# RustCrypto/elliptic-curves

Hardware: NVIDIA H100
Metric: scalar-mults/sec (var-base, batch) at 1/2/4/8 H100 vs reference Rust CPU (higher is better)
Workload: dtype u32

## Files before the change

__graft_entry__.py:

```python
import os
import subprocess
import sys

ROOT = os.path.dirname(os.path.abspath(__file__))
PKG = os.path.join(ROOT, "elliptic-curves_b200")
CSRC = os.path.join(PKG, "csrc")
LIB = os.path.join(PKG, "libecgpu.so")
NVCC_FLAGS = [
    "-gencode", "arch=compute_90a,code=sm_90a", "-O3", "-lineinfo", "-std=c++17",
    "-Xcompiler", "-fPIC",
]
CURVE_GROUPS = (0, 1, 2, 3, 4, 5, 6)


def _newer(target, sources):
    if not os.path.exists(target):
        return True
    t = os.path.getmtime(target)
    return any(os.path.getmtime(s) > t for s in sources)


def _paths():
    for p in (ROOT, PKG, os.path.join(ROOT, "oracle"), os.path.join(ROOT, "tests")):
        if p not in sys.path:
            sys.path.insert(0, p)


def _build_dev(nvcc, srcs, force):
    dev_dir = os.path.join(ROOT, "tests", "dev")
    src = os.path.join(dev_dir, "fe_dev.cu")
    dev_so, sim_so = os.path.join(dev_dir, "libecgdev.so"), os.path.join(dev_dir, "libecgdevsim.so")
    if force or _newer(sim_so, srcs + [src]):
        subprocess.check_call(["g++", "-O2", "-std=c++17", "-Wno-unknown-pragmas", "-shared", "-fPIC", "-x", "c++", "-o", sim_so, src])
    if force or _newer(dev_so, srcs + [src]):
        objdir = os.path.join(dev_dir, "_build")
        os.makedirs(objdir, exist_ok=True)
        procs, objs = [], []
        for part in ("0", "1", "2", "3", "4", None):
            obj = os.path.join(objdir, f"fe_dev_s{part}.o" if part else "fe_dev_main.o")
            cmd = [nvcc] + NVCC_FLAGS + ["-Xcompiler", "-fvisibility=hidden"] + ([f"-DDEV_SHAPE={part}"] if part else []) + ["-c", "-o", obj, src]
            print("[build]", " ".join(cmd), flush=True)
            procs.append((cmd, subprocess.Popen(cmd)))
            objs.append(obj)
        for cmd, pr in procs:
            if pr.wait() != 0:
                raise subprocess.CalledProcessError(pr.returncode, cmd)
        subprocess.check_call([nvcc, "-shared", "-o", dev_so] + objs)
    x_src = os.path.join(dev_dir, "x448_dev.cu")
    x_so, x_sim = os.path.join(dev_dir, "libecgx448dev.so"), os.path.join(dev_dir, "libecgx448devsim.so")
    if force or _newer(x_sim, srcs + [x_src]):
        subprocess.check_call(["g++", "-O2", "-std=c++17", "-Wno-unknown-pragmas", "-shared", "-fPIC", "-x", "c++", "-o", x_sim, x_src])
    if force or _newer(x_so, srcs + [x_src]):
        cmd = [nvcc] + NVCC_FLAGS + ["-Xcompiler", "-fvisibility=hidden", "-shared", "-o", x_so, x_src]
        print("[build]", " ".join(cmd), flush=True)
        subprocess.check_call(cmd)
    e_src = os.path.join(dev_dir, "ed448_dev.cu")
    e_so, e_sim = os.path.join(dev_dir, "libecged448dev.so"), os.path.join(dev_dir, "libecged448devsim.so")
    if force or _newer(e_sim, srcs + [e_src]):
        subprocess.check_call(["g++", "-O2", "-std=c++17", "-Wno-unknown-pragmas", "-shared", "-fPIC", "-x", "c++", "-o", e_sim, e_src])
    if force or _newer(e_so, srcs + [e_src]):
        cmd = [nvcc] + NVCC_FLAGS + ["-Xcompiler", "-fvisibility=hidden", "-shared", "-o", e_so, e_src]
        print("[build]", " ".join(cmd), flush=True)
        subprocess.check_call(cmd)
    g_src = os.path.join(dev_dir, "ed448_group_dev.cu")
    g_so, g_sim = os.path.join(dev_dir, "libecged448gdev.so"), os.path.join(dev_dir, "libecged448gdevsim.so")
    if force or _newer(g_sim, srcs + [g_src]):
        subprocess.check_call(["g++", "-O2", "-std=c++17", "-Wno-unknown-pragmas", "-shared", "-fPIC", "-x", "c++", "-o", g_sim, g_src])
    if force or _newer(g_so, srcs + [g_src]):
        cmd = [nvcc] + NVCC_FLAGS + ["-Xcompiler", "-fvisibility=hidden", "-shared", "-o", g_so, g_src]
        print("[build]", " ".join(cmd), flush=True)
        subprocess.check_call(cmd)


def build(force: bool = False) -> None:
    nvcc = os.environ.get("NVCC", "/usr/local/cuda/bin/nvcc")
    srcs = [os.path.join(CSRC, f) for f in sorted(os.listdir(CSRC))] + [os.path.join(ROOT, "include", "ecgpu.h")]
    if force or _newer(LIB, srcs):
        objdir = os.path.join(PKG, "_build")
        os.makedirs(objdir, exist_ok=True)
        procs, objs = [], []
        for g in CURVE_GROUPS:
            obj = os.path.join(objdir, f"ecgpu_tu{g}.o")
            cmd = [nvcc] + NVCC_FLAGS + [f"-DECG_TU={g}", "-c", "-o", obj, os.path.join(CSRC, "ecgpu.cu")]
            print("[build]", " ".join(cmd), flush=True)
            procs.append((cmd, subprocess.Popen(cmd)))
            objs.append(obj)
        for cmd, pr in procs:
            if pr.wait() != 0:
                raise subprocess.CalledProcessError(pr.returncode, cmd)
        cmd = [nvcc, "-shared", "-o", LIB] + objs
        print("[build]", " ".join(cmd), flush=True)
        subprocess.check_call(cmd)
    _paths()
    import ecref

    ecref.build(force)
    sim_dir = os.path.join(ROOT, "tests", "sim")
    sim_so = os.path.join(sim_dir, "libecgsim.so")
    if force or _newer(sim_so, srcs + [os.path.join(sim_dir, "sim.cpp")]):
        subprocess.check_call(["g++", "-O2", "-std=c++17", "-Wno-unknown-pragmas", "-shared", "-fPIC", "-pthread", "-o", sim_so,
                               os.path.join(sim_dir, "sim.cpp")])
    _build_dev(nvcc, srcs, force)
    import ecgpu

    ecgpu.load_library()


def smoke() -> None:
    _paths()
    if not os.path.exists(LIB):
        build()
    import numpy as np

    import ecgpu
    import ecref
    import pyref
    from helpers import pack_points, pack_scalars, random_points

    eng = ecgpu.Engine([0])
    for curve in ("k256", "p256"):
        c = pyref.CURVES[curve]
        n = 257
# ... 38 lines not shown
```

elliptic-curves_b200/csrc/ecg_fe_k256.cuh:

```cuda
#pragma once
#include "ecg_prim.cuh"

namespace ecg {

#ifndef ECG_K256_OPT
#define ECG_K256_OPT 7
#endif
#if defined(__CUDA_ARCH__) || defined(__CUDACC__)
#define ECG_NOINLINE_D __device__ __noinline__
#else
#define ECG_NOINLINE_D
#endif

template <int OPT>
struct FpK256T {
  static constexpr int NL = 8;
  static constexpr bool LE = false;
  static constexpr int FB = 32;
  typedef FeN<8> FeT;
  typedef JacN<8> JacT;
  typedef AffN<8> AffT;
  static constexpr uint32_t C0 = 977u;
  static constexpr bool SQR_TRADE_DBL = (OPT & 64) != 0;
  static constexpr bool SQR_TRADE_MADD = (OPT & 128) != 0;
  static constexpr bool DBL_CALL = (OPT & 2048) != 0;
  static constexpr bool MADD_CALL = (OPT & 4096) != 0;
  static constexpr bool DBL_3M5S = false;
  typedef FpK256T<(OPT & (1 | 8 | 64 | 128))> Inline;

  ECG_D static void set_zero(Fe& r) {
#pragma unroll
    for (int i = 0; i < 8; i++) r.v[i] = 0;
  }
  ECG_D static void set_one(Fe& r) {
    set_zero(r);
    r.v[0] = 1;
  }

  ECG_D static void fold_top(uint32_t* r, uint32_t t0, uint32_t t1) {
    uint32_t q0, q1;
    mul_wide(q0, q1, t0, C0);
    uint64_t s1 = (uint64_t)q1 + t0 + (t1 ? C0 : 0u);
    uint32_t p1 = (uint32_t)s1;
    uint32_t p2 = (uint32_t)(s1 >> 32) + t1;
    r[0] = add_cc(r[0], q0);
    r[1] = addc_cc(r[1], p1);
    r[2] = addc_cc(r[2], p2);
#pragma unroll
    for (int i = 3; i < 8; i++) r[i] = addc_cc(r[i], 0);
    uint32_t cf = addc(0, 0);
    r[0] = add_cc(r[0], cf ? C0 : 0u);
    r[1] = addc_cc(r[1], cf);
    r[2] = addc_cc(r[2], 0);
    r[3] = addc(r[3], 0);
  }

  ECG_D static void reduce16(Fe& r, const uint32_t* t) {
    uint32_t lo[8], q[8];
#pragma unroll
    for (int i = 0; i < 8; i++) {
      lo[i] = t[i];
      q[i] = t[8 + i];
    }
    mad_wide_cc(lo[0], lo[1], t[8], C0);
    madc_wide_cc(lo[2], lo[3], t[10], C0);
    madc_wide_cc(lo[4], lo[5], t[12], C0);
    madc_wide_cc(lo[6], lo[7], t[14], C0);
    uint32_t e8 = addc(0, 0);
    mad_wide_cc(q[0], q[1], t[9], C0);
    madc_wide_cc(q[2], q[3], t[11], C0);
    madc_wide_cc(q[4], q[5], t[13], C0);
    madc_wide_cc(q[6], q[7], t[15], C0);
    uint32_t q8 = addc(0, 0);
    r.v[0] = lo[0];
    r.v[1] = add_cc(lo[1], q[0]);
#pragma unroll
    for (int k = 2; k < 8; k++) r.v[k] = addc_cc(lo[k], q[k - 1]);
    uint32_t t0 = addc_cc(e8, q[7]);
    uint32_t t1 = addc(q8, 0);
    fold_top(r.v, t0, t1);
  }

  ECG_D static void mul_body(Fe& r, const Fe& a, const Fe& b) {
    uint32_t t[16];
    if (OPT & 8)
      mul8x8_kara(t, a.v, b.v);
    else
      mul8x8(t, a.v, b.v);
    reduce16(r, t);
  }
  ECG_D static void sqr_body(Fe& r, const Fe& a) {
    uint32_t t[16];
    if (OPT & 1)
      sqr8(t, a.v);
    else
      mul8x8(t, a.v, a.v);
    reduce16(r, t);
  }
  static ECG_NOINLINE_D Fe mul_call(Fe a, Fe b) {
    Fe r;
    mul_body(r, a, b);
    return r;
  }
  static ECG_NOINLINE_D void mul_call_mem(Fe* r, const Fe* a, const Fe* b) {
    Fe x = *a, y = *b, z;
    mul_body(z, x, y);
    *r = z;
  }
  static ECG_NOINLINE_D void sqr_call_mem(Fe* r, const Fe* a) {
    Fe x = *a, z;
    sqr_body(z, x);
    *r = z;
  }
  static ECG_NOINLINE_D Fe sqr_call(Fe a) {
    Fe r;
    sqr_body(r, a);
    return r;
  }
  ECG_D static void mul(Fe& r, const Fe& a, const Fe& b) {
    if (OPT & 256)
      mul_call_mem(&r, &a, &b);
    else if (OPT & 2)
      r = mul_call(a, b);
    else
      mul_body(r, a, b);
  }
  ECG_D static void mul_d(Fe& r, const Fe& a, const Fe& b) {
    if (OPT & 256)
      mul_call_mem(&r, &a, &b);
    else if ((OPT & 2) && !(OPT & 32))
      r = mul_call(a, b);
    else
      mul_body(r, a, b);
// ... 67 lines not shown
  ECG_D static bool is_zero(const Fe& a) {
    uint32_t o = a.v[0] | a.v[1] | a.v[2] | a.v[3] | a.v[4] | a.v[5] | a.v[6] | a.v[7];
    uint32_t n = (a.v[0] ^ 0xFFFFFC2Fu) | (a.v[1] ^ 0xFFFFFFFEu) | ~(a.v[2] & a.v[3] & a.v[4] & a.v[5] & a.v[6] & a.v[7]);
    return (o == 0) | (n == 0);
  }
  ECG_D static bool is_canonical(const Fe& a) {
    uint32_t hi = a.v[2] & a.v[3] & a.v[4] & a.v[5] & a.v[6] & a.v[7];
    bool ge = (hi == 0xFFFFFFFFu) && (a.v[1] == 0xFFFFFFFFu || (a.v[1] == 0xFFFFFFFEu && a.v[0] >= 0xFFFFFC2Fu));
    return !ge;
  }
  ECG_D static void sqr_n(Fe& r, const Fe& a, int n) {
    r = a;
#pragma unroll 1
    for (int i = 0; i < n; i++) sqr(r, r);
  }
  ECG_D static void inv(Fe& r, const Fe& a) {
    Fe x2, x3, x6, x9, x11, x22, x44, x88, x176, x220, x223, t;
    sqr(x2, a);
    mul(x2, x2, a);
    sqr(x3, x2);
    mul(x3, x3, a);
    sqr_n(x6, x3, 3);
    mul(x6, x6, x3);
    sqr_n(x9, x6, 3);
    mul(x9, x9, x3);
    sqr_n(x11, x9, 2);
    mul(x11, x11, x2);
    sqr_n(x22, x11, 11);
    mul(x22, x22, x11);
    sqr_n(x44, x22, 22);
    mul(x44, x44, x22);
    sqr_n(x88, x44, 44);
    mul(x88, x88, x44);
    sqr_n(x176, x88, 88);
    mul(x176, x176, x88);
    sqr_n(x220, x176, 44);
    mul(x220, x220, x44);
    sqr_n(x223, x220, 3);
    mul(x223, x223, x3);
    sqr_n(t, x223, 23);
    mul(t, t, x22);
    sqr_n(t, t, 5);
    mul(t, t, a);
    sqr_n(t, t, 3);
    mul(t, t, x2);
    sqr_n(t, t, 2);
    mul(r, t, a);
  }
  ECG_D static void from_canonical(Fe& r, const Fe& a) { r = a; }
  ECG_D static void to_canonical(Fe& r, const Fe& a) { normalize(r, a); }
};

typedef FpK256T<ECG_K256_OPT> FpK256;

}
```

elliptic-curves_b200/csrc/ecg_fe_mont.cuh:

```cuda
#pragma once
#include "ecg_prim.cuh"

namespace ecg {

#ifndef ECG_NOINLINE_D
#if defined(__CUDA_ARCH__) || defined(__CUDACC__)
#define ECG_NOINLINE_D __device__ __noinline__
#else
#define ECG_NOINLINE_D
#endif
#endif

template <class PR, bool CALLS = true>
struct FpMontT {
  static constexpr int NL = PR::NL;
  typedef PR Params;
  typedef FeN<NL> FeT;
  typedef JacN<NL> JacT;
  typedef AffN<NL> AffT;
  typedef FeT Fe;
  static constexpr bool MONT = true;
  static constexpr bool LE = PR::LE;
  static constexpr int FB = PR::FB;
  static constexpr bool SQR_TRADE_DBL = false;
  static constexpr bool SQR_TRADE_MADD = false;
  static constexpr bool DBL_CALL = false;
  static constexpr bool MADD_CALL = false;
  static constexpr bool DBL_3M5S = false;
  typedef FpMontT<PR, CALLS> Inline;

  ECG_D static void set_zero(Fe& r) {
#pragma unroll
    for (int i = 0; i < NL; i++) r.v[i] = 0;
  }
  ECG_D static void set_one(Fe& r) {
#pragma unroll
    for (int i = 0; i < NL; i++) r.v[i] = PR::ONE(i);
  }

  ECG_D static void cond_sub_p(Fe& r, const uint32_t* t, uint32_t carry) {
    uint32_t u[NL];
    u[0] = sub_cc(t[0], PR::P(0));
#pragma unroll
    for (int i = 1; i < NL; i++) u[i] = subc_cc(t[i], PR::P(i));
    uint32_t bw = 0u - subc(0u, 0u);
    bool take = (carry != 0) | (bw == 0);
#pragma unroll
    for (int i = 0; i < NL; i++) r.v[i] = take ? u[i] : t[i];
  }

  ECG_D static void redc_mersenne(Fe& r, const uint32_t* u) {
    constexpr int B = PR::MERSENNE, W = B / 32, S = B % 32, K = 32 * NL - B;
    static_assert(PR::MERSENNE == 0 || (W == NL - 1 && S > 0 && K == 32 - S), "one partial top limb");
    constexpr uint32_t TOPMASK = (1u << S) - 1u;
    uint32_t lo[NL], hi[NL], v[NL];
#pragma unroll
    for (int i = 0; i < W; i++) lo[i] = u[i];
    lo[W] = u[W] & TOPMASK;
#pragma unroll
    for (int i = 0; i < NL; i++) hi[i] = (u[W + i] >> S) | ((W + i + 1 < 2 * NL ? u[W + i + 1] : 0u) << K);
    addN<NL>(v, lo, hi);
    const uint32_t c = v[W] >> S;
    v[W] &= TOPMASK;
    v[0] = add_cc(v[0], c);
#pragma unroll
    for (int i = 1; i < NL - 1; i++) v[i] = addc_cc(v[i], 0u);
    v[NL - 1] = addc(v[NL - 1], 0u);
    Fe w;
    cond_sub_p(w, v, 0u);
    const uint32_t low = w.v[0] & ((1u << K) - 1u);
#pragma unroll
    for (int i = 0; i < W; i++) r.v[i] = (w.v[i] >> K) | (w.v[i + 1] << S);
    r.v[W] = 0;
    constexpr int POS = B - K, PL = POS / 32, PS = POS % 32;
    r.v[PL] |= low << PS;
    if (PS + K > 32) r.v[PL + 1] |= low >> (32 - PS);
  }
  ECG_D static void mul_full(uint32_t* u, const Fe& a, const Fe& b) {
// ... 211 lines not shown
```

elliptic-curves_b200/csrc/ecg_fe_p256.cuh:

```cuda
#pragma once
#include "ecg_prim.cuh"

namespace ecg {

#ifndef ECG_P256_OPT
#define ECG_P256_OPT 515
#endif
#ifndef ECG_NOINLINE_D
#if defined(__CUDA_ARCH__) || defined(__CUDACC__)
#define ECG_NOINLINE_D __device__ __noinline__
#else
#define ECG_NOINLINE_D
#endif
#endif

template <int OPT>
struct FpP256T {
  static constexpr int NL = 8;
  static constexpr bool LE = false;
  static constexpr int FB = 32;
  typedef FeN<8> FeT;
  typedef JacN<8> JacT;
  typedef AffN<8> AffT;
  static constexpr bool SQR_TRADE_DBL = false;
  static constexpr bool SQR_TRADE_MADD = false;
  static constexpr bool DBL_CALL = (OPT & 2048) != 0;
  static constexpr bool MADD_CALL = (OPT & 4096) != 0;
  static constexpr bool DBL_3M5S = (OPT & 1024) != 0;
  typedef FpP256T<(OPT & (1 | 8 | 16 | 512 | 1024))> Inline;
  ECG_D static void set_zero(Fe& r) {
#pragma unroll
    for (int i = 0; i < 8; i++) r.v[i] = 0;
  }
  static constexpr bool MONT = (OPT & 512) != 0;
  ECG_D static void set_one(Fe& r) {
    set_zero(r);
    r.v[0] = 1;
    if (MONT) {
      r.v[3] = r.v[4] = r.v[5] = 0xFFFFFFFFu;
      r.v[6] = 0xFFFFFFFEu;
    }
  }

  ECG_D static uint32_t add_K(uint32_t* r, uint32_t c) {
    uint32_t m = 0u - c;
    r[0] = add_cc(r[0], c);
    r[1] = addc_cc(r[1], 0);
    r[2] = addc_cc(r[2], 0);
    r[3] = addc_cc(r[3], m);
    r[4] = addc_cc(r[4], m);
    r[5] = addc_cc(r[5], m);
    r[6] = addc_cc(r[6], m & 0xFFFFFFFEu);
    r[7] = addc_cc(r[7], 0);
    return addc(0, 0);
  }
  ECG_D static uint32_t sub_K(uint32_t* r, uint32_t c) {
    uint32_t m = 0u - c;
    r[0] = sub_cc(r[0], c);
    r[1] = subc_cc(r[1], 0);
    r[2] = subc_cc(r[2], 0);
    r[3] = subc_cc(r[3], m);
    r[4] = subc_cc(r[4], m);
    r[5] = subc_cc(r[5], m);
    r[6] = subc_cc(r[6], m & 0xFFFFFFFEu);
    r[7] = subc_cc(r[7], 0);
    return 0u - subc(0, 0);
  }

  ECG_D static int32_t fold_signed(uint32_t* r, int32_t o) {
    int64_t t = (int64_t)r[0] + o;
    r[0] = (uint32_t)t;
    t >>= 32;
    t += r[1];
    r[1] = (uint32_t)t;
    t >>= 32;
    t += r[2];
    r[2] = (uint32_t)t;
    t >>= 32;
// ... 360 lines not shown
```

elliptic-curves_b200/csrc/ecg_fe_p384.cuh:

```cuda
#pragma once
#include "ecg_prim.cuh"

namespace ecg {

#ifndef ECG_P384_OPT
#define ECG_P384_OPT 2
#endif
#ifndef ECG_NOINLINE_D
#if defined(__CUDA_ARCH__) || defined(__CUDACC__)
#define ECG_NOINLINE_D __device__ __noinline__
#else
#define ECG_NOINLINE_D
#endif
#endif

template <int OPT>
struct FpP384T {
  static constexpr int NL = 12;
  static constexpr bool LE = false;
  static constexpr int FB = 48;
  typedef FeN<12> FeT;
  typedef JacN<12> JacT;
  typedef AffN<12> AffT;
  typedef FeT Fe;
  static constexpr bool MONT = false;
  static constexpr bool SQR_TRADE_DBL = false;
  static constexpr bool SQR_TRADE_MADD = false;
  static constexpr bool DBL_CALL = false;
  static constexpr bool MADD_CALL = false;
  static constexpr bool DBL_3M5S = false;
  typedef FpP384T<0> Inline;

  ECG_D static void set_zero(Fe& r) {
#pragma unroll
    for (int i = 0; i < 12; i++) r.v[i] = 0;
  }
  ECG_D static void set_one(Fe& r) {
    set_zero(r);
    r.v[0] = 1;
  }

  ECG_D static uint32_t add_oK(uint32_t* r, uint32_t o) {
    uint32_t m = o ? 0xFFFFFFFFu : 0u;
    r[0] = add_cc(r[0], o);
    r[1] = addc_cc(r[1], 0u - o);
    r[2] = addc_cc(r[2], m);
    r[3] = addc_cc(r[3], (o - 1u) & m);
    r[4] = addc_cc(r[4], o);
#pragma unroll
    for (int i = 5; i < 12; i++) r[i] = addc_cc(r[i], 0u);
    return addc(0u, 0u);
  }
  ECG_D static uint32_t sub_K(uint32_t* r, uint32_t c) {
    uint32_t m = 0u - c;
    r[0] = sub_cc(r[0], c);
    r[1] = subc_cc(r[1], m);
    r[2] = subc_cc(r[2], m);
    r[3] = subc_cc(r[3], 0u);
    r[4] = subc_cc(r[4], c);
#pragma unroll
    for (int i = 5; i < 12; i++) r[i] = subc_cc(r[i], 0u);
    return 0u - subc(0u, 0u);
  }

  ECG_D static void acc_add(uint32_t* acc, const uint32_t* v) {
    acc[0] = add_cc(acc[0], v[0]);
#pragma unroll
    for (int i = 1; i < 12; i++) acc[i] = addc_cc(acc[i], v[i]);
    acc[12] = addc(acc[12], 0u);
  }
  ECG_D static void acc_sub(uint32_t* acc, const uint32_t* v) {
    acc[0] = sub_cc(acc[0], v[0]);
#pragma unroll
    for (int i = 1; i < 12; i++) acc[i] = subc_cc(acc[i], v[i]);
    acc[12] = subc(acc[12], 0u);
  }

  ECG_D static void reduce24(Fe& r, const uint32_t* c) {
    uint32_t acc[13], v[12];
    acc[0] = add_cc(c[0], 0xFFFFFFFCu);
// ... 186 lines not shown
```

elliptic-curves_b200/csrc/ecg_kernels.cuh:

```cuda
#pragma once
#if defined(__CUDACC__)
#include <cuda_runtime.h>
#else
#ifndef ECG_HOST_SIM
#error "ecg_kernels.cuh is CUDA code; a host build exists only for the test simulation (tests/sim/sim.cpp)"
#endif
#endif

#include "../../include/ecgpu.h"
#include "ecg_curves.cuh"
#include "ecg_io.cuh"
#include "ecg_mul.cuh"
#include "ecg_verify.cuh"

using namespace ecg;

#define ERRF_SCALAR 1u
#define ERRF_POINT 2u
#define ERRF_SKEW 4u

ECG_DEV void report_error(uint32_t* status, uint32_t flag, size_t idx) {
  atomicOr(&status[0], flag);
  atomicMin(&status[1], (uint32_t)(idx > 0xFFFFFFFEull ? 0xFFFFFFFEull : idx));
}

template <int NW>
ECG_DEV void soa_store(uint32_t* buf, size_t n, size_t idx, const uint32_t* v, int w0) {
#pragma unroll
  for (int w = 0; w < NW; w++) buf[(size_t)(w0 + w) * n + idx] = v[w];
}
template <int NW>
ECG_DEV void soa_load(uint32_t* v, const uint32_t* buf, size_t n, size_t idx, int w0) {
#pragma unroll
  for (int w = 0; w < NW; w++) v[w] = buf[(size_t)(w0 + w) * n + idx];
}

template <class C>
ECG_DEV uint32_t load_pair(uint32_t* k, typename C::F::AffT& P, bool& inf, const uint8_t* kb,
                                              const uint8_t* pxy, const uint8_t* pinf, size_t idx) {
  typedef typename C::F F;
  typedef typename F::FeT Fe;
  constexpr int NL = F::NL, FB = F::FB;
  uint32_t err = 0;
  load_fe<F>(k, kb + FB * idx);
  if (!ltN<NL>(k, C::N())) err |= ERRF_SCALAR;
  inf = pinf != nullptr && pinf[idx] != 0;
  Fe x, y;
  load_fe<F>(x.v, pxy + 2 * FB * idx);
  load_fe<F>(y.v, pxy + 2 * FB * idx + FB);
  if (!inf) {
    bool ok = ltN<NL>(x.v, C::P()) && ltN<NL>(y.v, C::P());
    F::from_canonical(P.x, x);
    F::from_canonical(P.y, y);
    if (ok) {
      Fe b;
      C::b_internal(b);
      ok = aff_on_curve<F, C::A_IS_MINUS3>(P, b);
    }
    if (!ok) err |= ERRF_POINT;
  }
  if (inf || err) {
    C::generator(P);
#pragma unroll
    for (int i = 0; i < NL; i++) k[i] = (i == 0);
  }
  return err;
}

#define K_TAB_WORDS 128
#define P_TAB_WORDS 192

typedef FpK256T<1> FpK256Inline;
template <int BLOCK, int MINBLK>
ECG_KERNEL(BLOCK, MINBLK)
    k256_varbase_kernel(const uint8_t* __restrict__ kb, const uint8_t* __restrict__ pxy,
                        const uint8_t* __restrict__ pinf, size_t n, uint32_t* __restrict__ jac,
                        uint32_t* __restrict__ gtab, uint32_t* __restrict__ status, size_t base) {
  size_t idx = (size_t)blockIdx.x * BLOCK + threadIdx.x;
  const bool live = idx < n;
  const size_t cidx = live ? idx : n - 1;
  uint32_t k[8];
  Aff P;
  bool inf;
  uint32_t err = load_pair<CurveK256>(k, P, inf, kb, pxy, pinf, cidx);
  if (err && live) report_error(status, err, base + idx);
  TabRef tab{gtab + (size_t)blockIdx.x * BLOCK * K_TAB_WORDS + threadIdx.x, (uint32_t)BLOCK};
  Jac r;
  k256_mul_thread<FpK256Inline, 1>(r, k, P, tab);
  if (!live) return;
  if (inf || err) FpK256::set_zero(r.Z);
  soa_store<8>(jac, n, idx, r.X.v, 0);
  soa_store<8>(jac, n, idx, r.Y.v, 8);
  soa_store<8>(jac, n, idx, r.Z.v, 16);
}

template <class C>
ECG_DEV uint32_t load_pair_or_generator(uint32_t* k, typename C::F::AffT& P, bool& inf, const uint8_t* kb, const uint8_t* pxy,
                                        const uint8_t* pinf, size_t idx) {
  typedef typename C::F F;
  if (pxy != nullptr) return load_pair<C>(k, P, inf, kb, pxy, pinf, idx);
  inf = false;
  load_fe<F>(k, kb + F::FB * idx);
  C::generator(P);
  if (ltN<F::NL>(k, C::N())) return 0;
#pragma unroll
  for (int i = 0; i < F::NL; i++) k[i] = (i == 0);
  return ERRF_SCALAR;
}

template <int BLOCK, int MINBLK>
ECG_KERNEL(BLOCK, MINBLK)
    k256_varbase_ct_kernel(const uint8_t* __restrict__ kb, const uint8_t* __restrict__ pxy, const uint8_t* __restrict__ pinf, size_t n,
                           uint32_t* __restrict__ jac, uint32_t* __restrict__ gtab, uint32_t* __restrict__ status, size_t base) {
  size_t idx = (size_t)blockIdx.x * BLOCK + threadIdx.x;
  if (idx >= n) return;
  uint32_t k[8];
  Aff P;
  bool inf;
  uint32_t err = load_pair_or_generator<CurveK256>(k, P, inf, kb, pxy, pinf, idx);
  if (err) report_error(status, err, base + idx);
  TabRef tab{gtab + (size_t)blockIdx.x * BLOCK * K_TAB_WORDS + threadIdx.x, (uint32_t)BLOCK};
  Jac r;
  k256_mul_thread<FpK256, 0, true>(r, k, P, tab);
  if (inf || err) FpK256::set_zero(r.Z);
  soa_store<8>(jac, n, idx, r.X.v, 0);
  soa_store<8>(jac, n, idx, r.Y.v, 8);
  soa_store<8>(jac, n, idx, r.Z.v, 16);
}

template <class C, int BLOCK, int MINBLK, bool CT = false>
ECG_KERNEL(BLOCK, MINBLK)
    generic_varbase_kernel(const uint8_t* __restrict__ kb, const uint8_t* __restrict__ pxy,
                           const uint8_t* __restrict__ pinf, size_t n, uint32_t* __restrict__ jac,
                           uint32_t* __restrict__ gtab, uint32_t* __restrict__ status, size_t base) {
  typedef typename C::F F;
  constexpr int NL = F::NL;
  size_t idx = (size_t)blockIdx.x * BLOCK + threadIdx.x;
  if (idx >= n) return;
  uint32_t k[NL];
// ... 1007 lines not shown
```

elliptic-curves_b200/csrc/ecg_mul.cuh:

```cuda
#pragma once
#include "ecg_fe_k256.cuh"
#include "ecg_point.cuh"
#include "ecg_scalar.cuh"

namespace ecg {

template <int NL>
struct TabRefN {
  uint32_t* base;
  uint32_t stride;
  ECG_D void store(int e, const FeN<NL>& x, const FeN<NL>& y) const {
#pragma unroll
    for (int w = 0; w < NL; w++) {
      base[(e * 2 * NL + w) * stride] = x.v[w];
      base[(e * 2 * NL + NL + w) * stride] = y.v[w];
    }
  }
  ECG_D void load(int e, FeN<NL>& x, FeN<NL>& y) const {
#pragma unroll
    for (int w = 0; w < NL; w++) {
      x.v[w] = base[(e * 2 * NL + w) * stride];
      y.v[w] = base[(e * 2 * NL + NL + w) * stride];
    }
  }
  ECG_D void load_ct(uint32_t idx, FeN<NL>& x, FeN<NL>& y) const {
#pragma unroll
    for (int w = 0; w < NL; w++) x.v[w] = y.v[w] = 0;
#pragma unroll 1
    for (uint32_t e = 0; e < 8; e++) {
      const uint32_t m = 0u - (uint32_t)(e == idx);
#pragma unroll
      for (int w = 0; w < NL; w++) {
        x.v[w] |= base[(e * 2 * NL + w) * stride] & m;
        y.v[w] |= base[(e * 2 * NL + NL + w) * stride] & m;
      }
    }
  }
};
typedef TabRefN<8> TabRef;
template <int NL>
struct TabRefJN {
  uint32_t* base;
  uint32_t stride;
  ECG_D void store(int e, const JacN<NL>& p) const {
#pragma unroll
    for (int w = 0; w < NL; w++) {
      base[(e * 3 * NL + w) * stride] = p.X.v[w];
      base[(e * 3 * NL + NL + w) * stride] = p.Y.v[w];
      base[(e * 3 * NL + 2 * NL + w) * stride] = p.Z.v[w];
    }
  }
  ECG_D void load(int e, JacN<NL>& p) const {
#pragma unroll
    for (int w = 0; w < NL; w++) {
      p.X.v[w] = base[(e * 3 * NL + w) * stride];
      p.Y.v[w] = base[(e * 3 * NL + NL + w) * stride];
      p.Z.v[w] = base[(e * 3 * NL + 2 * NL + w) * stride];
    }
  }
  ECG_D void load_ct(uint32_t idx, JacN<NL>& p) const {
#pragma unroll
    for (int w = 0; w < NL; w++) p.X.v[w] = p.Y.v[w] = p.Z.v[w] = 0;
#pragma unroll 1
    for (uint32_t e = 0; e < 8; e++) {
      const uint32_t m = 0u - (uint32_t)(e == idx);
#pragma unroll
      for (int w = 0; w < NL; w++) {
        p.X.v[w] |= base[(e * 3 * NL + w) * stride] & m;
        p.Y.v[w] |= base[(e * 3 * NL + NL + w) * stride] & m;
        p.Z.v[w] |= base[(e * 3 * NL + 2 * NL + w) * stride] & m;
      }
    }
  }
};
typedef TabRefJN<8> TabRefJ;

ECG_D void k256_beta(Fe& b) {
  const uint32_t B[8] = {0x719501EEu, 0xC1396C28u, 0x12F58995u, 0x9CF04975u, 0xAC3434E9u, 0x6E64479Eu, 0x657C0710u, 0x7AE96A2Bu};
#pragma unroll
  for (int i = 0; i < 8; i++) b.v[i] = B[i];
}

template <class F>
ECG_D void build_table_iso_a0(const TabRef& tab, Fe& Zg, const Aff& P) {
  Jac d, cur;
  aff_dbl<F, false>(d, P);
  Fe z2, z3;
  F::sqr(z2, d.Z);
  F::mul(z3, z2, d.Z);
  F::mul(cur.X, P.x, z2);
  F::mul(cur.Y, P.y, z3);
  F::set_one(cur.Z);
  Aff dd;
  dd.x = d.X;
  dd.y = d.Y;
  Fe zr[8];
  tab.store(0, cur.X, cur.Y);
#pragma unroll 1
  for (int i = 1; i < 8; i++) {
    jac_madd<F, false>(cur, cur, dd, &zr[i]);
    tab.store(i, cur.X, cur.Y);
  }
  F::mul(Zg, cur.Z, d.Z);
  Fe zs = zr[7];
#pragma unroll 1
  for (int i = 6; i >= 0; i--) {
    Fe x, y, zz;
    tab.load(i, x, y);
    F::sqr(zz, zs);
    F::mul(x, x, zz);
    F::mul(zz, zz, zs);
    F::mul(y, y, zz);
    tab.store(i, x, y);
    if (i > 0) F::mul(zs, zs, zr[i]);
  }
}

#if defined(__CUDA_ARCH__)
#define ECG_BLOCK_SYNC() __syncthreads()
#else
#define ECG_BLOCK_SYNC() ((void)0)
#endif
template <class F = FpK256, int PHASE_SYNC = 0, bool CT = false>
ECG_D void k256_mul_thread(Jac& r, const uint32_t* k, const Aff& P, const TabRef& tab) {
  GlvHalf g1, g2;
  glv_split_k256<CT>(g1, g2, k);
  Fe Zg, beta;
  build_table_iso_a0<F>(tab, Zg, P);
  k256_beta(beta);

  Jac acc;
  Aff e;
  tab.load(0, acc.X, acc.Y);
  fe_cneg<F>(acc.Y, g1.neg);
  F::set_one(acc.Z);
  tab.load(0, e.x, e.y);
  F::mul(e.x, e.x, beta);
  fe_cneg<F>(e.y, g2.neg);
  jac_madd<F, false>(acc, acc, e);

#pragma unroll 1
  for (int i = 0; i < 32; i++) {
    if (PHASE_SYNC == 1) ECG_BLOCK_SYNC();
#pragma unroll 1
    for (int j = 0; j < 4; j++) {
      if (PHASE_SYNC == 2) ECG_BLOCK_SYNC();
      jac_dbl<F, false>(acc, acc);
    }
    if (PHASE_SYNC == 1) ECG_BLOCK_SYNC();
#pragma unroll 1
    for (int half = 0; half < 2; half++) {
      if (PHASE_SYNC == 2) ECG_BLOCK_SYNC();
      uint32_t n = half ? next_window(g2.h) : next_window(g1.h);
      uint32_t sneg = half ? g2.neg : g1.neg;
      uint32_t pos = n >> 3;
      uint32_t idx = pos ? (n & 7u) : (7u - n);
      if (CT)
        tab.load_ct(idx, e.x, e.y);
      else
        tab.load((int)idx, e.x, e.y);
      if (half) F::mul(e.x, e.x, beta);
      fe_cneg<F>(e.y, (pos ^ sneg) ^ 1u);
      jac_madd<F, false>(acc, acc, e);
    }
  }
#pragma unroll 1
  for (int half = 0; half < 2; half++) {
    uint32_t ev = half ? g2.even : g1.even;
    uint32_t sneg = half ? g2.neg : g1.neg;
    tab.load(0, e.x, e.y);
    if (half) F::mul(e.x, e.x, beta);
    fe_cneg<F>(e.y, sneg ^ 1u);
    Jac t;
    jac_madd<F, false>(t, acc, e);
    jac_csel(acc, t, ev);
  }
  r.X = acc.X;
  r.Y = acc.Y;
  F::mul(r.Z, acc.Z, Zg);
}

template <class F, int A_IS_MINUS3, int PHASE_SYNC = 0, bool CT = false>
ECG_D void generic_mul_thread(typename F::JacT& r, const uint32_t* k, const typename F::AffT& P, const TabRefJN<F::NL>& tab) {
  typedef typename F::JacT Jac;
  typedef typename F::AffT Aff;
  FullRecodeN<F::NL> rc;
  recode_full<F::NL>(rc, k);
  Jac d, cur, acc;
  aff_dbl<F, A_IS_MINUS3>(d, P);
  cur.X = P.x;
  cur.Y = P.y;
  F::set_one(cur.Z);
  acc = cur;
  tab.store(0, cur);
  jac_madd<F, A_IS_MINUS3>(cur, d, P);
  tab.store(1, cur);
#pragma unroll 1
  for (int i = 2; i < 8; i++) {
    jac_add<F, A_IS_MINUS3>(cur, cur, d);
    tab.store(i, cur);
  }
#pragma unroll 1
  for (int i = 0; i < F::NL * 8; i++) {
#pragma unroll 1
    for (int j = 0; j < 4; j++) {
      if (PHASE_SYNC == 2) ECG_BLOCK_SYNC();
      jac_dbl<F, A_IS_MINUS3>(acc, acc);
    }
    if (PHASE_SYNC == 2) ECG_BLOCK_SYNC();
    uint32_t n = next_windowN<F::NL>(rc.h);
    uint32_t pos = n >> 3;
    uint32_t idx = pos ? (n & 7u) : (7u - n);
    Jac e;
    if (CT)
      tab.load_ct(idx, e);
    else
      tab.load((int)idx, e);
    fe_cneg<F>(e.Y, pos ^ 1u);
    jac_add<F, A_IS_MINUS3>(acc, acc, e);
  }
  Aff np;
  np.x = P.x;
  F::neg(np.y, P.y);
  Jac t;
// ... 7 lines not shown
```

elliptic-curves_b200/csrc/ecg_point.cuh:

```cuda
#pragma once
#include "ecg_prim.cuh"

namespace ecg {

typedef JacN<8> Jac;
typedef AffN<8> Aff;

template <class F>
ECG_D void fe_cneg(typename F::FeT& a, uint32_t c) {
  typename F::FeT n;
  F::neg(n, a);
#pragma unroll
  for (int i = 0; i < F::NL; i++) a.v[i] = c ? n.v[i] : a.v[i];
}
template <int NL>
ECG_D void jac_csel(JacN<NL>& r, const JacN<NL>& t, uint32_t c) {
#pragma unroll
  for (int i = 0; i < NL; i++) {
    r.X.v[i] = c ? t.X.v[i] : r.X.v[i];
    r.Y.v[i] = c ? t.Y.v[i] : r.Y.v[i];
    r.Z.v[i] = c ? t.Z.v[i] : r.Z.v[i];
  }
}

template <class F, int A_IS_MINUS3>
ECG_D void jac_dbl_body(typename F::JacT& r, const typename F::JacT& p) {
  typedef typename F::FeT Fe;
  Fe A, L, T, D, t, zz;
  F::sqr(A, p.Y);
  if (A_IS_MINUS3 == 1) {
    Fe u, v;
    F::sqr(zz, p.Z);
    F::sub(u, p.X, zz);
    F::add(v, p.X, zz);
    F::mul_d(L, u, v);
  } else {
    F::sqr(L, p.X);
  }
  F::sqr(D, A);
  if (A_IS_MINUS3 == 0 && F::SQR_TRADE_DBL) {
    F::add(t, p.X, A);
    F::sqr(T, t);
    F::sub(T, T, L);
    F::sub(T, T, D);
    F::half(T, T);
  } else {
    F::mul_d(T, p.X, A);
  }
  F::mul_small(L, L, 3);
  if constexpr (A_IS_MINUS3 == 2) {
    Fe z4, ca;
    F::sqr(zz, p.Z);
    F::sqr(z4, zz);
    F::curve_a(ca);
    F::mul_d(z4, z4, ca);
    F::add(L, L, z4);
  }
  F::half(L, L);
  if (A_IS_MINUS3 == 1 && F::DBL_3M5S) {
    Fe s2;
    F::add(s2, p.Y, p.Z);
    F::sqr(s2, s2);
    F::sub(s2, s2, A);
    F::sub(s2, s2, zz);
    F::half(r.Z, s2);
  } else {
    F::mul_d(r.Z, p.Y, p.Z);
  }
  F::sqr(r.X, L);
  F::add(t, T, T);
  F::sub(r.X, r.X, t);
  F::sub(t, T, r.X);
  F::mul_d(r.Y, L, t);
  F::sub(r.Y, r.Y, D);
}

#if defined(__CUDA_ARCH__) || defined(__CUDACC__)
#define ECG_NOINLINE_PT __device__ __noinline__
#else
#define ECG_NOINLINE_PT
#endif
template <class F, int A_IS_MINUS3>
ECG_NOINLINE_PT typename F::JacT jac_dbl_call(typename F::JacT p) {
  typename F::JacT r;
  jac_dbl_body<typename F::Inline, A_IS_MINUS3>(r, p);
  return r;
}
template <class F, int A_IS_MINUS3>
ECG_D void jac_dbl(typename F::JacT& r, const typename F::JacT& p) {
  if (F::DBL_CALL)
    r = jac_dbl_call<F, A_IS_MINUS3>(p);
  else
    jac_dbl_body<F, A_IS_MINUS3>(r, p);
}

template <class F, int A_IS_MINUS3>
ECG_D void aff_dbl(typename F::JacT& r, const typename F::AffT& p) {
  typename F::JacT j;
  j.X = p.x;
  j.Y = p.y;
  F::set_one(j.Z);
  jac_dbl<F, A_IS_MINUS3>(r, j);
}

template <class F, int A_IS_MINUS3>
#if defined(__CUDA_ARCH__)
__device__ __noinline__
#else
inline
#endif
    void
    jac_madd_slow(typename F::JacT& r, const typename F::JacT& p, const typename F::AffT& q, bool z1zero, bool rzero) {
  if (z1zero) {
    r.X = q.x;
    r.Y = q.y;
    F::set_one(r.Z);
  } else if (rzero) {
    aff_dbl<F, A_IS_MINUS3>(r, q);
  } else {
    F::set_zero(r.X);
    F::set_one(r.Y);
    F::set_zero(r.Z);
  }
}

template <class F, int A_IS_MINUS3>
ECG_D void jac_madd_body(typename F::JacT& r, const typename F::JacT& p, const typename F::AffT& q, typename F::FeT* zr = nullptr) {
  typedef typename F::FeT Fe;
  Fe zz, u2, s2, H, R, hh, hhh, V, t;
  F::sqr(zz, p.Z);
  F::mul(u2, q.x, zz);
  F::mul(s2, p.Z, zz);
  F::mul(s2, s2, q.y);
  F::sub(H, u2, p.X);
  F::sub(R, s2, p.Y);
  bool z1zero = F::is_zero(p.Z);
  bool hzero = F::is_zero(H);
  if (z1zero | hzero) {
    jac_madd_slow<F, A_IS_MINUS3>(r, p, q, z1zero, F::is_zero(R));
    if (zr) F::set_zero(*zr);
    return;
  }
  F::sqr(hh, H);
  F::mul(hhh, H, hh);
  F::mul(V, p.X, hh);
  if (F::SQR_TRADE_MADD) {
    F::add(t, p.Z, H);
    F::sqr(t, t);
    F::sub(t, t, zz);
    F::sub(t, t, hh);
    F::half(r.Z, t);
  } else {
    F::mul(r.Z, p.Z, H);
  }
  if (zr) *zr = H;
  F::sqr(t, R);
  F::sub(t, t, hhh);
  F::sub(t, t, V);
  F::sub(r.X, t, V);
  F::sub(t, V, r.X);
  F::mul(t, t, R);
  F::mul(hhh, hhh, p.Y);
  F::sub(r.Y, t, hhh);
}

template <class F, int A_IS_MINUS3>
ECG_NOINLINE_PT typename F::JacT jac_madd_call(typename F::JacT p, typename F::AffT q) {
  typename F::JacT r;
  jac_madd_body<typename F::Inline, A_IS_MINUS3>(r, p, q, nullptr);
  return r;
}
template <class F, int A_IS_MINUS3>
ECG_D void jac_madd(typename F::JacT& r, const typename F::JacT& p, const typename F::AffT& q, typename F::FeT* zr = nullptr) {
  if (F::MADD_CALL && zr == nullptr)
    r = jac_madd_call<F, A_IS_MINUS3>(p, q);
  else
    jac_madd_body<F, A_IS_MINUS3>(r, p, q, zr);
}

template <class F, int A_IS_MINUS3>
ECG_D void jac_add(typename F::JacT& r, const typename F::JacT& p, const typename F::JacT& q) {
  typedef typename F::FeT Fe;
  bool z1zero = F::is_zero(p.Z), z2zero = F::is_zero(q.Z);
  if (z1zero) {
    r = q;
    return;
  }
  if (z2zero) {
    r = p;
    return;
  }
  Fe z1z1, z2z2, u1, u2, s1, s2, H, R, hh, hhh, V, t;
  F::sqr(z1z1, p.Z);
  F::sqr(z2z2, q.Z);
  F::mul(u1, p.X, z2z2);
  F::mul(u2, q.X, z1z1);
  F::mul(s1, q.Z, z2z2);
  F::mul(s1, s1, p.Y);
  F::mul(s2, p.Z, z1z1);
  F::mul(s2, s2, q.Y);
  F::sub(H, u2, u1);
  F::sub(R, s2, s1);
  if (F::is_zero(H)) {
    if (F::is_zero(R)) {
      jac_dbl<F, A_IS_MINUS3>(r, p);
    } else {
      F::set_zero(r.X);
      F::set_one(r.Y);
      F::set_zero(r.Z);
    }
    return;
  }
  F::sqr(hh, H);
  F::mul(hhh, H, hh);
  F::mul(V, u1, hh);
  F::mul(t, p.Z, q.Z);
// ... 34 lines not shown
```

Measured before the change: 52.45 million.

## Add beta-column table, fused mul-sub reduction, and half-add tripling for k256

For the k256 variable-base kernel, the precomputed table gains a third column holding x*beta, so GLV second-half lookups no longer need a field multiplication per addition. The table grows from 128 to 192 words per thread, raising global-memory traffic and footprint. Doubling and mixed addition also fuse 'a*b - c*d' (and 'a*b - c^2') into a single shared reduction via a borrow-corrected 512-bit subtraction, saving one modular reduction each. Tripling followed by halving is replaced with a half-then-add sequence.

```diff
diff --git a/__graft_entry__.py b/__graft_entry__.py
--- a/__graft_entry__.py
+++ b/__graft_entry__.py
@@ -68,6 +68,14 @@
         subprocess.check_call(["g++", "-O2", "-std=c++17", "-Wno-unknown-pragmas", "-shared", "-fPIC", "-x", "c++", "-o", g_sim, g_src])
     if force or _newer(g_so, srcs + [g_src]):
         cmd = [nvcc] + NVCC_FLAGS + ["-Xcompiler", "-fvisibility=hidden", "-shared", "-o", g_so, g_src]
+        print("[build]", " ".join(cmd), flush=True)
+        subprocess.check_call(cmd)
+    l_src = os.path.join(dev_dir, "k256_lean_dev.cu")
+    l_so, l_sim = os.path.join(dev_dir, "libecgk256leandev.so"), os.path.join(dev_dir, "libecgk256leandevsim.so")
+    if force or _newer(l_sim, srcs + [l_src]):
+        subprocess.check_call(["g++", "-O2", "-std=c++17", "-Wno-unknown-pragmas", "-shared", "-fPIC", "-x", "c++", "-o", l_sim, l_src])
+    if force or _newer(l_so, srcs + [l_src]):
+        cmd = [nvcc] + NVCC_FLAGS + ["-Xcompiler", "-fvisibility=hidden", "-shared", "-o", l_so, l_src]
         print("[build]", " ".join(cmd), flush=True)
         subprocess.check_call(cmd)
 
diff --git a/elliptic-curves_b200/csrc/ecg_fe_k256.cuh b/elliptic-curves_b200/csrc/ecg_fe_k256.cuh
--- a/elliptic-curves_b200/csrc/ecg_fe_k256.cuh
+++ b/elliptic-curves_b200/csrc/ecg_fe_k256.cuh
@@ -26,7 +26,10 @@
   static constexpr bool DBL_CALL = (OPT & 2048) != 0;
   static constexpr bool MADD_CALL = (OPT & 4096) != 0;
   static constexpr bool DBL_3M5S = false;
-  typedef FpK256T<(OPT & (1 | 8 | 64 | 128))> Inline;
+  static constexpr bool BETA_COLUMN = (OPT & 8192) != 0;
+  static constexpr bool HALF3_ADD = (OPT & 16384) != 0;
+  static constexpr bool MUL_SUB = (OPT & 32768) != 0;
+  typedef FpK256T<(OPT & (1 | 8 | 64 | 128 | 8192 | 16384 | 32768))> Inline;
 
   ECG_D static void set_zero(Fe& r) {
 #pragma unroll
@@ -37,13 +40,15 @@
     r.v[0] = 1;
   }
 
-  ECG_D static void fold_top(uint32_t* r, uint32_t t0, uint32_t t1) {
+  ECG_D static void fold_top(uint32_t* r, uint32_t t0, uint32_t t1, uint32_t e = 0) {
     uint32_t q0, q1;
     mul_wide(q0, q1, t0, C0);
-    uint64_t s1 = (uint64_t)q1 + t0 + (t1 ? C0 : 0u);
+    uint64_t s0 = (uint64_t)q0 + (e ? 954529u : 0u);
+    uint64_t s1 = (uint64_t)q1 + t0 + (t1 ? C0 : 0u) + (e ? 1954u : 0u) + (s0 >> 32);
+    uint32_t q0s = (uint32_t)s0;
     uint32_t p1 = (uint32_t)s1;
-    uint32_t p2 = (uint32_t)(s1 >> 32) + t1;
-    r[0] = add_cc(r[0], q0);
+    uint32_t p2 = (uint32_t)(s1 >> 32) + t1 + e;
+    r[0] = add_cc(r[0], q0s);
     r[1] = addc_cc(r[1], p1);
     r[2] = addc_cc(r[2], p2);
 #pragma unroll
@@ -55,7 +60,7 @@
     r[3] = addc(r[3], 0);
   }
 
-  ECG_D static void reduce16(Fe& r, const uint32_t* t) {
+  ECG_D static void reduce16(Fe& r, const uint32_t* t, uint32_t e = 0) {
     uint32_t lo[8], q[8];
 #pragma unroll
     for (int i = 0; i < 8; i++) {
@@ -78,7 +83,40 @@
     for (int k = 2; k < 8; k++) r.v[k] = addc_cc(lo[k], q[k - 1]);
     uint32_t t0 = addc_cc(e8, q[7]);
     uint32_t t1 = addc(q8, 0);
-    fold_top(r.v, t0, t1);
+    fold_top(r.v, t0, t1, e);
+  }
+  ECG_D static void sub_reduce16(Fe& r, uint32_t* t, const uint32_t* u) {
+    const uint32_t bw = subN<16>(t, t, u);
+    const uint32_t m = 0u - bw;
+    t[8] = sub_cc(t[8], m & 1954u);
+    t[9] = subc_cc(t[9], m & 2u);
+#pragma unroll
+    for (int i = 10; i < 16; i++) t[i] = subc_cc(t[i], 0);
+    const uint32_t b2 = 0u - subc(0, 0);
+    reduce16(r, t, bw ^ b2);
+  }
+  ECG_D static void mul_sub(Fe& r, const Fe& a, const Fe& b, const Fe& c, const Fe& d) {
+    uint32_t t[16], u[16];
+    if (OPT & 8) {
+      mul8x8_kara(u, c.v, d.v);
+      mul8x8_kara(t, a.v, b.v);
+    } else {
+      mul8x8(u, c.v, d.v);
+      mul8x8(t, a.v, b.v);
+    }
+    sub_reduce16(r, t, u);
+  }
+  ECG_D static void mul_sub_sqr(Fe& r, const Fe& a, const Fe& b, const Fe& c) {
+    uint32_t t[16], u[16];
+    if (OPT & 1)
+      sqr8(u, c.v);
+    else
+      mul8x8(u, c.v, c.v);
+    if (OPT & 8)
+      mul8x8_kara(t, a.v, b.v);
+    else
+      mul8x8(t, a.v, b.v);
+    sub_reduce16(r, t, u);
   }
 
   ECG_D static void mul_body(Fe& r, const Fe& a, const Fe& b) {
@@ -252,5 +290,6 @@
 };
 
 typedef FpK256T<ECG_K256_OPT> FpK256;
+typedef FpK256T<1 | 8192 | 16384 | 32768> FpK256Inline;
 
 }
diff --git a/elliptic-curves_b200/csrc/ecg_fe_mont.cuh b/elliptic-curves_b200/csrc/ecg_fe_mont.cuh
--- a/elliptic-curves_b200/csrc/ecg_fe_mont.cuh
+++ b/elliptic-curves_b200/csrc/ecg_fe_mont.cuh
@@ -24,6 +24,7 @@
   static constexpr int FB = PR::FB;
   static constexpr bool SQR_TRADE_DBL = false;
   static constexpr bool SQR_TRADE_MADD = false;
+  static constexpr bool HALF3_ADD = false, MUL_SUB = false;
   static constexpr bool DBL_CALL = false;
   static constexpr bool MADD_CALL = false;
   static constexpr bool DBL_3M5S = false;
diff --git a/elliptic-curves_b200/csrc/ecg_fe_p256.cuh b/elliptic-curves_b200/csrc/ecg_fe_p256.cuh
--- a/elliptic-curves_b200/csrc/ecg_fe_p256.cuh
+++ b/elliptic-curves_b200/csrc/ecg_fe_p256.cuh
@@ -24,6 +24,7 @@
   typedef AffN<8> AffT;
   static constexpr bool SQR_TRADE_DBL = false;
   static constexpr bool SQR_TRADE_MADD = false;
+  static constexpr bool HALF3_ADD = false, MUL_SUB = false;
   static constexpr bool DBL_CALL = (OPT & 2048) != 0;
   static constexpr bool MADD_CALL = (OPT & 4096) != 0;
   static constexpr bool DBL_3M5S = (OPT & 1024) != 0;
diff --git a/elliptic-curves_b200/csrc/ecg_fe_p384.cuh b/elliptic-curves_b200/csrc/ecg_fe_p384.cuh
--- a/elliptic-curves_b200/csrc/ecg_fe_p384.cuh
+++ b/elliptic-curves_b200/csrc/ecg_fe_p384.cuh
@@ -26,6 +26,7 @@
   static constexpr bool MONT = false;
   static constexpr bool SQR_TRADE_DBL = false;
   static constexpr bool SQR_TRADE_MADD = false;
+  static constexpr bool HALF3_ADD = false, MUL_SUB = false;
   static constexpr bool DBL_CALL = false;
   static constexpr bool MADD_CALL = false;
   static constexpr bool DBL_3M5S = false;
diff --git a/elliptic-curves_b200/csrc/ecg_kernels.cuh b/elliptic-curves_b200/csrc/ecg_kernels.cuh
--- a/elliptic-curves_b200/csrc/ecg_kernels.cuh
+++ b/elliptic-curves_b200/csrc/ecg_kernels.cuh
@@ -67,10 +67,9 @@
   return err;
 }
 
-#define K_TAB_WORDS 128
+#define K_TAB_WORDS 192
 #define P_TAB_WORDS 192
 
-typedef FpK256T<1> FpK256Inline;
 template <int BLOCK, int MINBLK>
 ECG_KERNEL(BLOCK, MINBLK)
     k256_varbase_kernel(const uint8_t* __restrict__ kb, const uint8_t* __restrict__ pxy,
@@ -84,7 +83,7 @@
   bool inf;
   uint32_t err = load_pair<CurveK256>(k, P, inf, kb, pxy, pinf, cidx);
   if (err && live) report_error(status, err, base + idx);
-  TabRef tab{gtab + (size_t)blockIdx.x * BLOCK * K_TAB_WORDS + threadIdx.x, (uint32_t)BLOCK};
+  K256TabRef<FpK256Inline> tab{gtab + (size_t)blockIdx.x * BLOCK * K_TAB_WORDS + threadIdx.x, (uint32_t)BLOCK};
   Jac r;
   k256_mul_thread<FpK256Inline, 1>(r, k, P, tab);
   if (!live) return;
diff --git a/elliptic-curves_b200/csrc/ecg_mul.cuh b/elliptic-curves_b200/csrc/ecg_mul.cuh
--- a/elliptic-curves_b200/csrc/ecg_mul.cuh
+++ b/elliptic-curves_b200/csrc/ecg_mul.cuh
@@ -5,25 +5,30 @@
 
 namespace ecg {
 
-template <int NL>
+template <int NL, int WPE = 2 * NL>
 struct TabRefN {
   uint32_t* base;
   uint32_t stride;
   ECG_D void store(int e, const FeN<NL>& x, const FeN<NL>& y) const {
 #pragma unroll
     for (int w = 0; w < NL; w++) {
-      base[(e * 2 * NL + w) * stride] = x.v[w];
-      base[(e * 2 * NL + NL + w) * stride] = y.v[w];
-    }
-  }
-  ECG_D void load(int e, FeN<NL>& x, FeN<NL>& y) const {
-#pragma unroll
-    for (int w = 0; w < NL; w++) {
-      x.v[w] = base[(e * 2 * NL + w) * stride];
-      y.v[w] = base[(e * 2 * NL + NL + w) * stride];
+      base[(e * WPE + w) * stride] = x.v[w];
+      base[(e * WPE + NL + w) * stride] = y.v[w];
+    }
+  }
+  ECG_D void store_x2(int e, const FeN<NL>& x2) const {
+#pragma unroll
+    for (int w = 0; w < NL; w++) base[(e * WPE + 2 * NL + w) * stride] = x2.v[w];
+  }
+  ECG_D void load(int e, FeN<NL>& x, FeN<NL>& y, int xcol = 0) const {
+#pragma unroll
+    for (int w = 0; w < NL; w++) {
+      x.v[w] = base[(e * WPE + xcol + w) * stride];
+      y.v[w] = base[(e * WPE + NL + w) * stride];
     }
   }
   ECG_D void load_ct(uint32_t idx, FeN<NL>& x, FeN<NL>& y) const {
+    static_assert(WPE == 2 * NL, "the masked scan covers the (x, y) layout only");
 #pragma unroll
     for (int w = 0; w < NL; w++) x.v[w] = y.v[w] = 0;
 #pragma unroll 1
@@ -31,13 +36,15 @@
       const uint32_t m = 0u - (uint32_t)(e == idx);
 #pragma unroll
       for (int w = 0; w < NL; w++) {
-        x.v[w] |= base[(e * 2 * NL + w) * stride] & m;
-        y.v[w] |= base[(e * 2 * NL + NL + w) * stride] & m;
+        x.v[w] |= base[(e * WPE + w) * stride] & m;
+        y.v[w] |= base[(e * WPE + NL + w) * stride] & m;
       }
     }
   }
 };
 typedef TabRefN<8> TabRef;
+template <class F>
+using K256TabRef = TabRefN<8, F::BETA_COLUMN ? 24 : 16>;
 template <int NL>
 struct TabRefJN {
   uint32_t* base;
@@ -82,7 +89,7 @@
 }
 
 template <class F>
-ECG_D void build_table_iso_a0(const TabRef& tab, Fe& Zg, const Aff& P) {
+ECG_D void build_table_iso_a0(const K256TabRef<F>& tab, Fe& Zg, const Aff& P) {
   Jac d, cur;
   aff_dbl<F, false>(d, P);
   Fe z2, z3;
@@ -102,7 +109,12 @@
     tab.store(i, cur.X, cur.Y);
   }
   F::mul(Zg, cur.Z, d.Z);
-  Fe zs = zr[7];
+  Fe zs = zr[7], beta;
+  if constexpr (F::BETA_COLUMN) {
+    k256_beta(beta);
+    F::mul(cur.X, cur.X, beta);
+    tab.store_x2(7, cur.X);
+  }
 #pragma unroll 1
   for (int i = 6; i >= 0; i--) {
     Fe x, y, zz;
@@ -112,6 +124,10 @@
     F::mul(zz, zz, zs);
     F::mul(y, y, zz);
     tab.store(i, x, y);
+    if constexpr (F::BETA_COLUMN) {
+      F::mul(x, x, beta);
+      tab.store_x2(i, x);
+    }
     if (i > 0) F::mul(zs, zs, zr[i]);
   }
 }
@@ -122,20 +138,21 @@
 #define ECG_BLOCK_SYNC() ((void)0)
 #endif
 template <class F = FpK256, int PHASE_SYNC = 0, bool CT = false>
-ECG_D void k256_mul_thread(Jac& r, const uint32_t* k, const Aff& P, const TabRef& tab) {
+ECG_D void k256_mul_thread(Jac& r, const uint32_t* k, const Aff& P, const K256TabRef<F>& tab) {
   GlvHalf g1, g2;
   glv_split_k256<CT>(g1, g2, k);
   Fe Zg, beta;
   build_table_iso_a0<F>(tab, Zg, P);
   k256_beta(beta);
+  constexpr int BX = F::BETA_COLUMN ? 16 : 0;
 
   Jac acc;
   Aff e;
   tab.load(0, acc.X, acc.Y);
   fe_cneg<F>(acc.Y, g1.neg);
   F::set_one(acc.Z);
-  tab.load(0, e.x, e.y);
-  F::mul(e.x, e.x, beta);
+  tab.load(0, e.x, e.y, BX);
+  if (!F::BETA_COLUMN) F::mul(e.x, e.x, beta);
   fe_cneg<F>(e.y, g2.neg);
   jac_madd<F, false>(acc, acc, e);
 
@@ -155,11 +172,16 @@
       uint32_t sneg = half ? g2.neg : g1.neg;
       uint32_t pos = n >> 3;
       uint32_t idx = pos ? (n & 7u) : (7u - n);
-      if (CT)
-        tab.load_ct(idx, e.x, e.y);
-      else
-        tab.load((int)idx, e.x, e.y);
-      if (half) F::mul(e.x, e.x, beta);
+      if constexpr (F::BETA_COLUMN) {
+        static_assert(!CT, "the masked scan reads the (x, y) layout");
+        tab.load((int)idx, e.x, e.y, half ? BX : 0);
+      } else {
+        if (CT)
+          tab.load_ct(idx, e.x, e.y);
+        else
+          tab.load((int)idx, e.x, e.y);
+        if (half) F::mul(e.x, e.x, beta);
+      }
       fe_cneg<F>(e.y, (pos ^ sneg) ^ 1u);
       jac_madd<F, false>(acc, acc, e);
     }
@@ -168,8 +190,8 @@
   for (int half = 0; half < 2; half++) {
     uint32_t ev = half ? g2.even : g1.even;
     uint32_t sneg = half ? g2.neg : g1.neg;
-    tab.load(0, e.x, e.y);
-    if (half) F::mul(e.x, e.x, beta);
+    tab.load(0, e.x, e.y, half ? BX : 0);
+    if (half && !F::BETA_COLUMN) F::mul(e.x, e.x, beta);
     fe_cneg<F>(e.y, sneg ^ 1u);
     Jac t;
     jac_madd<F, false>(t, acc, e);
diff --git a/elliptic-curves_b200/csrc/ecg_point.cuh b/elliptic-curves_b200/csrc/ecg_point.cuh
--- a/elliptic-curves_b200/csrc/ecg_point.cuh
+++ b/elliptic-curves_b200/csrc/ecg_point.cuh
@@ -37,7 +37,8 @@
   } else {
     F::sqr(L, p.X);
   }
-  F::sqr(D, A);
+  constexpr bool Y3_MUL_SUB = A_IS_MINUS3 == 0 && F::MUL_SUB && !F::SQR_TRADE_DBL;
+  if constexpr (!Y3_MUL_SUB) F::sqr(D, A);
   if (A_IS_MINUS3 == 0 && F::SQR_TRADE_DBL) {
     F::add(t, p.X, A);
     F::sqr(T, t);
@@ -47,16 +48,21 @@
   } else {
     F::mul_d(T, p.X, A);
   }
-  F::mul_small(L, L, 3);
-  if constexpr (A_IS_MINUS3 == 2) {
-    Fe z4, ca;
-    F::sqr(zz, p.Z);
-    F::sqr(z4, zz);
-    F::curve_a(ca);
-    F::mul_d(z4, z4, ca);
-    F::add(L, L, z4);
-  }
-  F::half(L, L);
+  if constexpr (A_IS_MINUS3 == 0 && F::HALF3_ADD) {
+    F::half(t, L);
+    F::add(L, L, t);
+  } else {
+    F::mul_small(L, L, 3);
+    if constexpr (A_IS_MINUS3 == 2) {
+      Fe z4, ca;
+      F::sqr(zz, p.Z);
+      F::sqr(z4, zz);
+      F::curve_a(ca);
+      F::mul_d(z4, z4, ca);
+      F::add(L, L, z4);
+    }
+    F::half(L, L);
+  }
   if (A_IS_MINUS3 == 1 && F::DBL_3M5S) {
     Fe s2;
     F::add(s2, p.Y, p.Z);
@@ -71,8 +77,12 @@
   F::add(t, T, T);
   F::sub(r.X, r.X, t);
   F::sub(t, T, r.X);
-  F::mul_d(r.Y, L, t);
-  F::sub(r.Y, r.Y, D);
+  if constexpr (Y3_MUL_SUB) {
+    F::mul_sub_sqr(r.Y, L, t, A);
+  } else {
+    F::mul_d(r.Y, L, t);
+    F::sub(r.Y, r.Y, D);
+  }
 }
 
 #if defined(__CUDA_ARCH__) || defined(__CUDACC__)
@@ -159,9 +169,13 @@
   F::sub(t, t, V);
   F::sub(r.X, t, V);
   F::sub(t, V, r.X);
-  F::mul(t, t, R);
-  F::mul(hhh, hhh, p.Y);
-  F::sub(r.Y, t, hhh);
+  if constexpr (F::MUL_SUB) {
+    F::mul_sub(r.Y, t, R, hhh, p.Y);
+  } else {
+    F::mul(t, t, R);
+    F::mul(hhh, hhh, p.Y);
+    F::sub(r.Y, t, hhh);
+  }
 }
 
 template <class F, int A_IS_MINUS3>
```

Measured after the change: 54.90 million (median of 6 runs). +4.7%, better.
